# huziqi/NALO-SLAM

Measured on AMD Instinct MI355X. Metric: keyframes/sec, KITTI-00 dense 8-KF photometric BA; pose RMSE vs ref, higher is better.
Workload: dtype f32; 1 GPU; kitti00_8kf; image=1224x368, levels=4, window_frames=8, active_points=2000, residuals=14000, tracked_frames_per_keyframe=3, multi_gpu=replicas (window too small to shard)

## Files before the change

### nalo-slam_amd/csrc/kernels_tracker.hip

```cpp
#include "nalo_internal.h"
#include "reduce.h"
#include "trk_device.h"

namespace nalo {

struct TrkEvalParams {
    TrkLevel L;
    int lvl;
    int i0, i1;
    float RKi[9], t[3], Ki[9];
    float affa, affb, b0, cutoff, maxEnergy;
};
typedef float trk_f4 __attribute__((ext_vector_type(4)));

constexpr int kTrkEvalNT = 512;
constexpr int kTrkEvalNG = kTrkEvalNT / 13;
__global__ __launch_bounds__(kTrkEvalNT) void trk_eval_kernel(TrkEvalParams P, float* __restrict__ partial, unsigned* __restrict__ ticket, double* __restrict__ out, double seq) {
    __shared__ __attribute__((aligned(16))) float smem[(kTrkEvalNT / 4) * (kTrkVals + 1)];
    float acc[kTrkVals];
#pragma unroll
    for (int k = 0; k < kTrkVals; ++k) acc[k] = 0.f;
    const TrkLevel& L = P.L;
    const float wlm3 = (float)(L.wl - 3), hlm3 = (float)(L.hl - 3);
    for (int i = P.i0 + blockIdx.x * blockDim.x + threadIdx.x; i < P.i1; i += gridDim.x * blockDim.x) {
// ... 69 lines not shown
int trk_eval_launch(nalo_ctx* c, int slot_new, int lvl, const float RKi[9], const float t[3], const float Ki[9],
                    float affa, float affb, float b0, float cutoff, float maxEnergy, double out64[64]) {
    TrkEvalParams P;
    P.L = trk_level(c, slot_new, lvl); P.lvl = lvl;
    const bool sharded = c->trk_world > 1 && c->trk_hook;
    P.i0 = sharded ? (int)((long long)P.L.n * c->trk_rank / c->trk_world) : 0;
    P.i1 = sharded ? (int)((long long)P.L.n * (c->trk_rank + 1) / c->trk_world) : P.L.n;
    for (int i = 0; i < 9; ++i) { P.RKi[i] = RKi[i]; P.Ki[i] = Ki[i]; }
    for (int i = 0; i < 3; ++i) P.t[i] = t[i];
    P.affa = affa; P.affb = affb; P.b0 = b0; P.cutoff = cutoff; P.maxEnergy = maxEnergy;
    int nblocks = (P.i1 - P.i0 + kTrkEvalNT - 1) / kTrkEvalNT;
    nblocks = nblocks < 1 ? 1 : (nblocks > 512 ? 512 : nblocks);
    NALO_HIP(c, c->trk_partial.reserve((size_t)2048 * 64));
    if (!c->trk_ticket.p) { NALO_HIP(c, c->trk_ticket.reserve(4)); NALO_HIP(c, hipMemsetAsync(c->trk_ticket.p, 0, 16, c->stream)); }
    double* const dout = c->trk_out_host.dev;
    const double seq = (double)(++c->trk_seq);
    if (sharded) NALO_HIP(c, c->trk_shard_sums.reserve(64));
    {
        ProfScope ps(c, "trk_eval");
        trk_eval_kernel<<<nblocks, kTrkEvalNT, 0, c->stream>>>(P, c->trk_partial.p, c->trk_ticket.p, sharded ? c->trk_shard_sums.p : dout, sharded ? 0.0 : seq);
    }
    if (sharded) {
        if (!c->trk_hook_stream_ordered) NALO_HIP(c, hipStreamSynchronize(c->stream));
        c->trk_hook(c->trk_hook_user, c->trk_shard_sums.p, kTrkVals);
        if (c->xchg_failed) return NALO_ERR_HIP;
        trk_publish_kernel<<<1, 64, 0, c->stream>>>(c->trk_shard_sums.p, dout, seq);
    }
    NALO_HIP(c, hipGetLastError());
    if (!poll_flag(c, &c->trk_out_host.p[63], seq)) return NALO_ERR_HIP;
    std::memcpy(out64, c->trk_out_host.p, sizeof(double) * kTrkVals);
    return NALO_OK;
}

__global__ __launch_bounds__(256) void trk_scatter_kernel(const float* __restrict__ Ku, const float* __restrict__ Kv, const float* __restrict__ nid,
                                                          const float* __restrict__ HdiF, int n, int w0, int h0, float* __restrict__ idepth, float* __restrict__ wsum, int* __restrict__ cnt) {
    const int i = blockIdx.x * blockDim.x + threadIdx.x;
    if (i >= n) return;
    const int u = (int)(Ku[i] + 0.5f), v = (int)(Kv[i] + 0.5f);
    if (u < 0 || v < 0 || u >= w0 || v >= h0) return;
    const float weight = sqrtf((float)(1e-3 / ((double)HdiF[i] + 1e-12)));
    atomicAdd(idepth + u + w0 * v, nid[i] * weight);
    atomicAdd(wsum + u + w0 * v, weight);
    atomicAdd(cnt + u + w0 * v, 1);
}
constexpr int kScatterFixLds = 4096;
struct ScatterListLds {
    int* p;
    __device__ int ld(int k) const { return p[k]; }
    __device__ void st(int k, int v) const { p[k] = v; }
};
struct ScatterListGlobal {
    int* p;
    __device__ int ld(int k) const { return __hip_atomic_load(p + k, __ATOMIC_RELAXED, __HIP_MEMORY_SCOPE_AGENT); }
    __device__ void st(int k, int v) const { __hip_atomic_store(p + k, v, __ATOMIC_RELAXED, __HIP_MEMORY_SCOPE_AGENT); }
};
template <int NT, class List>
__device__ __forceinline__ void trk_scatter_fix_rounds(List list, int m, const float* __restrict__ Ku, const float* __restrict__ Kv, const float* __restrict__ nid,
                                                       const float* __restrict__ HdiF, int w0, float* __restrict__ idepth, float* __restrict__ wsum, int* __restrict__ cnt) {
    const int tid = threadIdx.x;
    for (int k = tid; k < m; k += NT) {
        const int i = list.ld(k), p = (int)(Ku[i] + 0.5f) + w0 * (int)(Kv[i] + 0.5f);
        atomicExch(idepth + p, 0.f); atomicExch(wsum + p, 0.f); atomicExch(cnt + p, 0x7fffffff);
    }
    __syncthreads();
    for (int k = tid; k < m; k += NT) { const int i = list.ld(k); atomicMin(cnt + (int)(Ku[i] + 0.5f) + w0 * (int)(Kv[i] + 0.5f), i); }
    __syncthreads();
    for (int round = 0; round < m; ++round) {
        bool any = false;
        for (int k = tid; k < m; k += NT) {
            const int i = list.ld(k);
            if (i < 0) continue;
            const int p = (int)(Ku[i] + 0.5f) + w0 * (int)(Kv[i] + 0.5f);
            if (__hip_atomic_load(cnt + p, __ATOMIC_RELAXED, __HIP_MEMORY_SCOPE_AGENT) == i) {
                const float weight = sqrtf((float)(1e-3 / ((double)HdiF[i] + 1e-12)));
                atomicAdd(idepth + p, __fmul_rn(nid[i], weight)); atomicAdd(wsum + p, weight);
                list.st(k, -1 - i);
            } else any = true;
        }
        __syncthreads();
        if (!__syncthreads_or(any)) break;
        for (int k = tid; k < m; k += NT) { const int i = list.ld(k); if (i < 0) { const int j = -1 - i, p = (int)(Ku[j] + 0.5f) + w0 * (int)(Kv[j] + 0.5f); atomicCAS(cnt + p, j, 0x7fffffff); } }
        __syncthreads();
        for (int k = tid; k < m; k += NT) { const int i = list.ld(k); if (i >= 0) atomicMin(cnt + (int)(Ku[i] + 0.5f) + w0 * (int)(Kv[i] + 0.5f), i); }
        __syncthreads();
    }
}
template <int NT>
__device__ __forceinline__ void trk_scatter_fix_body(const float* __restrict__ Ku, const float* __restrict__ Kv, const float* __restrict__ nid, const float* __restrict__ HdiF,
                                                     int w0, float* __restrict__ idepth, float* __restrict__ wsum, int* __restrict__ cnt, int* __restrict__ hot, int* slist) {
    const int tid = threadIdx.x;
    const int m = __hip_atomic_load(hot, __ATOMIC_RELAXED, __HIP_MEMORY_SCOPE_AGENT);
    if (m == 0) return;
    __syncthreads();
    if (tid == 0) __hip_atomic_store(hot, 0, __ATOMIC_RELAXED, __HIP_MEMORY_SCOPE_AGENT);
    if (m > kScatterFixLds) { trk_scatter_fix_rounds<NT>(ScatterListGlobal{hot + 2}, m, Ku, Kv, nid, HdiF, w0, idepth, wsum, cnt); return; }
    for (int k = tid; k < m; k += NT) slist[k] = __hip_atomic_load(hot + 2 + k, __ATOMIC_RELAXED, __HIP_MEMORY_SCOPE_AGENT);
    __syncthreads();
    trk_scatter_fix_rounds<NT>(ScatterListLds{slist}, m, Ku, Kv, nid, HdiF, w0, idepth, wsum, cnt);
}
__global__ __launch_bounds__(256) void trk_scatter_hot_kernel(const float* __restrict__ Ku, const float* __restrict__ Kv, const float* __restrict__ nid, const float* __restrict__ HdiF,
                                                              int n, int w0, int h0, float* __restrict__ idepth, float* __restrict__ wsum, int* __restrict__ cnt,
                                                              int* __restrict__ hot ) {
    __shared__ int slist[kScatterFixLds];
    __shared__ int is_last;
    const int i = blockIdx.x * blockDim.x + threadIdx.x;
    if (i < n) {
        const int u = (int)(Ku[i] + 0.5f), v = (int)(Kv[i] + 0.5f);
        if (!(u < 0 || v < 0 || u >= w0 || v >= h0) && __hip_atomic_load(cnt + u + w0 * v, __ATOMIC_RELAXED, __HIP_MEMORY_SCOPE_AGENT) >= 3) {
            const int at = atomicAdd(hot, 1);
            __hip_atomic_store(hot + 2 + at, i, __ATOMIC_RELAXED, __HIP_MEMORY_SCOPE_AGENT);
        }
    }
    __builtin_amdgcn_fence(__ATOMIC_RELEASE, "workgroup");
    __syncthreads();
    if (threadIdx.x == 0) is_last = __hip_atomic_fetch_add((unsigned*)(hot + 1), 1u, __ATOMIC_RELAXED, __HIP_MEMORY_SCOPE_AGENT) == gridDim.x - 1u;
    __syncthreads();
    if (!is_last) return;
    if (threadIdx.x == 0) __hip_atomic_store(hot + 1, 0, __ATOMIC_RELAXED, __HIP_MEMORY_SCOPE_AGENT);
    trk_scatter_fix_body<256>(Ku, Kv, nid, HdiF, w0, idepth, wsum, cnt, hot, slist);
}
struct TrkLevels {
    float *id[NALO_MAX_LEVELS], *ws[NALO_MAX_LEVELS], *wb[NALO_MAX_LEVELS];
    const float4* dI[NALO_MAX_LEVELS];
    float *pu[NALO_MAX_LEVELS], *pv[NALO_MAX_LEVELS], *pid[NALO_MAX_LEVELS], *pcol[NALO_MAX_LEVELS];
    int wl[NALO_MAX_LEVELS], hl[NALO_MAX_LEVELS];
    int blk0[NALO_MAX_LEVELS + 1];
    int scan0[NALO_MAX_LEVELS + 1];
    int L;
};
__global__ __launch_bounds__(256) void trk_zero2_kernel(float* __restrict__ a, float* __restrict__ b, int* __restrict__ cnt, int n) {
    const int i = blockIdx.x * blockDim.x + threadIdx.x;
    if (i < n) { a[i] = 0.f; b[i] = 0.f; cnt[i] = 0; }
    if (i == 0) { cnt[n] = 0; cnt[n + 1] = 0; }
}
__global__ __launch_bounds__(256) void trk_sum_down_all_kernel(TrkLevels P) {
    __shared__ float sid[2][16 * 16], sws[2][16 * 16];
    const int tx = threadIdx.x & 15, ty = threadIdx.x >> 4;
    const int tiles_x = (P.wl[1] + 15) / 16;
    const int bx = blockIdx.x % tiles_x, by = blockIdx.x / tiles_x;
    {
        const int x = bx * 16 + tx, y = by * 16 + ty, w0 = P.wl[0];
        float a = 0.f, b = 0.f;
        if (x < P.wl[1] && y < P.hl[1]) {
            const int o = 2 * x + 2 * y * w0;
            a = P.id[0][o] + P.id[0][o + 1] + P.id[0][o + w0] + P.id[0][o + w0 + 1];
            b = P.ws[0][o] + P.ws[0][o + 1] + P.ws[0][o + w0] + P.ws[0][o + w0 + 1];
            P.id[1][x + y * P.wl[1]] = a; P.ws[1][x + y * P.wl[1]] = b;
        }
        sid[0][ty * 16 + tx] = a; sws[0][ty * 16 + tx] = b;
    }
    int side = 16, cur = 0;
    for (int l = 2; l < P.L; ++l) {
        __syncthreads();
        const int ps = side; side >>= 1;
        if (side == 0) break;
        if (tx < side && ty < side) {
            const int x = bx * side + tx, y = by * side + ty, o = 2 * tx + 2 * ty * ps;
            const float a = sid[cur][o] + sid[cur][o + 1] + sid[cur][o + ps] + sid[cur][o + ps + 1];
            const float b = sws[cur][o] + sws[cur][o + 1] + sws[cur][o + ps] + sws[cur][o + ps + 1];
            if (x < P.wl[l] && y < P.hl[l]) { P.id[l][x + y * P.wl[l]] = a; P.ws[l][x + y * P.wl[l]] = b; }
            sid[cur ^ 1][ty * side + tx] = a; sws[cur ^ 1][ty * side + tx] = b;
        }
        cur ^= 1;
    }
}
__global__ __launch_bounds__(256) void trk_dilate_all_kernel(TrkLevels P) {
    int l = 0;
    while (l + 1 < P.L && (int)blockIdx.x >= P.blk0[l + 1]) ++l;
    const int wl = P.wl[l], npx = wl * P.hl[l];
    const int i = (blockIdx.x - P.blk0[l]) * blockDim.x + threadIdx.x;
    if (i >= npx) return;
    float* __restrict__ id = P.id[l]; const float* __restrict__ bak = P.ws[l]; float* __restrict__ out = P.wb[l];
    const float own = bak[i];
    float res = own;
    if (i >= wl && i < npx - wl && !(own > 0)) {
        const int diag = l < 2;
        const int o0 = diag ? 1 + wl : 1, o1 = diag ? -1 - wl : -1, o2 = diag ? wl - 1 : wl, o3 = diag ? -wl + 1 : -wl;
        float sum = 0, num = 0, numn = 0;
#define NALO_TAP(o) { const int j = i + (o); if (j >= 0 && j < npx) { const float b = bak[j]; if (b > 0) { sum += id[j]; num += b; numn++; } } }
        NALO_TAP(o0) NALO_TAP(o1) NALO_TAP(o2) NALO_TAP(o3)
#undef NALO_TAP
        if (numn > 0) { id[i] = sum / numn; res = num / numn; }
    }
    out[i] = res;
}
constexpr int kCompactChunk = 2048;
template <int WRITE>
__global__ __launch_bounds__(256) void trk_compact_all_kernel(TrkLevels P, int* __restrict__ scan) {
    constexpr int R = kCompactChunk / 256;
    __shared__ int cnt[R * 4 + 1];
    int l = 0;
    while (l + 1 < P.L && (int)blockIdx.x >= P.blk0[l + 1]) ++l;
    const int chunk = blockIdx.x - P.blk0[l], nb = P.blk0[l + 1] - P.blk0[l];
    const int wl = P.wl[l], hl = P.hl[l];
    float* __restrict__ id = P.id[l]; float* __restrict__ ws = P.wb[l]; const float4* __restrict__ dIref = P.dI[l];
    int* counts = scan + P.scan0[l]; const int* offsets = counts + nb;
    const int iw = wl - 4, ih = hl - 4, total = iw * ih;
    const int base = chunk * kCompactChunk;
    const int lane = threadIdx.x & 63, wave = threadIdx.x >> 6;
    int idx[R]; float wsv[R];
#pragma unroll
    for (int r = 0; r < R; ++r) {
        const int e = base + r * 256 + threadIdx.x;
        idx[r] = -1; wsv[r] = 0.f;
        if (e < total) { const int y = e / iw, x = e - y * iw; idx[r] = (x + 2) + (y + 2) * wl; wsv[r] = ws[idx[r]]; }
    }
    float val[R], col[R]; bool keep[R];
#pragma unroll
    for (int r = 0; r < R; ++r) {
        val[r] = 0.f; col[r] = 0.f; keep[r] = false;
        if (idx[r] >= 0 && wsv[r] > 0) { val[r] = id[idx[r]]; col[r] = dIref[idx[r]].x; }
    }
    int rank[R];
#pragma unroll
    for (int r = 0; r < R; ++r) {
        if (idx[r] >= 0 && wsv[r] > 0) { val[r] = val[r] / wsv[r]; keep[r] = isfinite(col[r]) && (val[r] > 0); }
        const unsigned long long m = __ballot(keep[r]);
        rank[r] = __popcll(m & ((1ull << lane) - 1ull));
        if (lane == 0) cnt[r * 4 + wave] = __popcll(m);
    }
    __syncthreads();
    if (!WRITE) {
        if (threadIdx.x == 0) { int t = 0; for (int k = 0; k < R * 4; ++k) t += cnt[k]; counts[chunk] = t; }
        return;
    }
    if (threadIdx.x < 64) {
        const int v = lane < R * 4 ? cnt[lane] : 0;
        int inc = v;
#pragma unroll
        for (int o = 1; o < 64; o <<= 1) { const int t = __shfl_up(inc, o); if (lane >= o) inc += t; }
        if (lane < R * 4) cnt[lane] = inc - v;
    }
    __syncthreads();
    const int first = offsets[chunk];
#pragma unroll
    for (int r = 0; r < R; ++r) {
        const int i = idx[r];
        if (i < 0) continue;
        if (wsv[r] > 0) {
            id[i] = keep[r] ? val[r] : -1.f; if (keep[r]) ws[i] = 1.f;
            if (keep[r]) {
                const int o = first + cnt[r * 4 + wave] + rank[r];
                const int y = i / wl, x = i - y * wl;
                P.pu[l][o] = (float)x; P.pv[l][o] = (float)y; P.pid[l][o] = val[r]; P.pcol[l][o] = col[r];
            }
        } else { id[i] = -1.f; ws[i] = 1.f; }
    }
}
__global__ __launch_bounds__(1024) void trk_scan_all_kernel(TrkLevels P, int* __restrict__ scan, double* __restrict__ out, double seq) {
    __shared__ int part[4][4];
    const int grp = threadIdx.x >> 8, t = threadIdx.x & 255, lane = threadIdx.x & 63, wave = t >> 6;
    for (int l0 = 0; l0 < P.L; l0 += 4) {
        const int l = l0 + grp;
        const bool on = l < P.L;
        const int nb = on ? P.blk0[l + 1] - P.blk0[l] : 0;
        const int* counts = scan + (on ? P.scan0[l] : 0); int* offsets = scan + (on ? P.scan0[l] : 0) + nb;
        const int per = (nb + 255) / 256, lo = min(t * per, nb), hi = min(lo + per, nb);
        int s = 0;
        for (int i = lo; i < hi; ++i) s += counts[i];
        int v = s;
#pragma unroll
        for (int off = 1; off < 64; off <<= 1) { const int nbv = __shfl_up(v, off); if (lane >= off) v += nbv; }
        if (lane == 63) part[grp][wave] = v;
        __syncthreads();
        int wpre = 0, tot = 0;
        for (int k = 0; k < 4; ++k) { const int pv = part[grp][k]; if (k < wave) wpre += pv; tot += pv; }
        int run = wpre + v - s;
        for (int i = lo; i < hi; ++i) { offsets[i] = run; run += counts[i]; }
        if (on && t == 0) { offsets[nb] = tot; out[l] = (double)tot; }
        __syncthreads();
    }
    __threadfence_system();
    __syncthreads();
    if (threadIdx.x == 0) __hip_atomic_store(&out[NALO_MAX_LEVELS], seq, __ATOMIC_RELEASE, __HIP_MEMORY_SCOPE_SYSTEM);
}

__global__ __launch_bounds__(1024) void trk_append_plane_kernel(const float* __restrict__ mask, const float4* __restrict__ dIref, int w, float d0, float d1, float d2, float dis,
                                                                float Ki00, float Ki02, float Ki11, float Ki12, float refColor, int x0, int nx, int y0, int ny, int n0,
                                                                float* __restrict__ pu, float* __restrict__ pv, float* __restrict__ pid, float* __restrict__ pcol, int* __restrict__ n_out) {
    __shared__ int wave_cnt[16];
    __shared__ int base_s;
    const int tid = threadIdx.x, lane = tid & 63, wv = tid >> 6;
    if (tid == 0) { base_s = 0; pu[n0] = 0.f; pv[n0] = 0.f; pid[n0] = 0.f; pcol[n0] = 0.f; }
    __syncthreads();
    const float t0 = d0 * Ki00 + d1 * 0.f + d2 * 0.f, t1 = d0 * 0.f + d1 * Ki11 + d2 * 0.f, t2 = d0 * Ki02 + d1 * Ki12 + d2 * 1.f;
    const int total = nx * ny;
    for (int c0 = 0; c0 < total; c0 += 1024) {
        const int j = c0 + tid;
        bool take = false; int x = 0, y = 0;
        if (j < total) { x = x0 + 5 * (j / ny); y = y0 + 5 * (j % ny); take = mask[x + y * w] == refColor; }
        const unsigned long long b = __ballot(take);
        if (lane == 0) wave_cnt[wv] = __popcll(b);
        __syncthreads();
        int off = base_s;
        for (int k = 0; k < wv; ++k) off += wave_cnt[k];
        if (take) {
            const int at = n0 + 1 + off + __popcll(b & ((1ull << lane) - 1ull));
            float nid = t0 * (float)x + t1 * (float)y + t2 * 1.f;
            nid /= -dis;
            pu[at] = (float)x; pv[at] = (float)y; pid[at] = nid; pcol[at] = dIref[x + y * w].x;
        }
        __syncthreads();
        if (tid == 0) { int s = 0; for (int k = 0; k < 16; ++k) s += wave_cnt[k]; base_s += s; }
        __syncthreads();
    }
    if (tid == 0) *n_out = base_s;
}
int trk_append_plane_launch(nalo_ctx* c, const float* mask, const float4* dIref, const float dir[3], float dis, float refColor, int x0, int nx, int y0, int ny, int n0, int* n_dev) {
    const float fx = c->fx[0], fy = c->fy[0], cx = c->cx[0], cy = c->cy[0];
    trk_append_plane_kernel<<<1, 1024, 0, c->stream>>>(mask, dIref, c->w, dir[0], dir[1], dir[2], dis, 1.0f / fx, -cx / fx, 1.0f / fy, -cy / fy, refColor, x0, nx, y0, ny, n0,
                                                       c->pc_u[0].p, c->pc_v[0].p, c->pc_id[0].p, c->pc_col[0].p, n_dev);
    NALO_HIP(c, hipGetLastError());
    return NALO_OK;
}

int trk_build_ref(nalo_ctx* c, int n, const float* dKu, const float* dKv, const float* dId, const float* dHdi) {
    const int L = c->levels;
    TrkLevels P;
    std::memset(&P, 0, sizeof(P));
    P.L = L;
    int dil_blocks = 0, cmp_blocks = 0, scan_total = 0;
    int dil0[NALO_MAX_LEVELS + 1] = {0}, cmp0[NALO_MAX_LEVELS + 1] = {0};
    for (int l = 0; l < L; ++l) {
        const size_t npx = (size_t)c->wl[l] * c->hl[l];
        NALO_HIP(c, c->trk_idepth[l].reserve(npx)); NALO_HIP(c, c->trk_wsum[l].reserve(npx)); NALO_HIP(c, c->trk_wbak[l].reserve(npx));
        NALO_HIP(c, c->pc_u[l].reserve(npx)); NALO_HIP(c, c->pc_v[l].reserve(npx)); NALO_HIP(c, c->pc_id[l].reserve(npx)); NALO_HIP(c, c->pc_col[l].reserve(npx));
        P.id[l] = c->trk_idepth[l].p; P.ws[l] = c->trk_wsum[l].p; P.wb[l] = c->trk_wbak[l].p; P.dI[l] = c->slots[c->slot_ref].dI[l].p;
        P.pu[l] = c->pc_u[l].p; P.pv[l] = c->pc_v[l].p; P.pid[l] = c->pc_id[l].p; P.pcol[l] = c->pc_col[l].p;
        P.wl[l] = c->wl[l]; P.hl[l] = c->hl[l];
        dil0[l] = dil_blocks; dil_blocks += (int)((npx + 255) / 256);
        const int total = (c->wl[l] - 4) * (c->hl[l] - 4);
        const int nb = total > 0 ? (total + kCompactChunk - 1) / kCompactChunk : 0;
        cmp0[l] = cmp_blocks; cmp_blocks += nb;
        P.scan0[l] = scan_total; scan_total += 2 * nb + 2;
    }
    dil0[L] = dil_blocks; cmp0[L] = cmp_blocks; P.scan0[L] = scan_total;
    NALO_HIP(c, c->scan_tmp.reserve((size_t)scan_total));
    const int n0 = c->wl[0] * c->hl[0];
    NALO_HIP(c, c->trk_cnt.reserve((size_t)n0 + 2 + std::max(n, 0)));
    trk_zero2_kernel<<<(n0 + 255) / 256, 256, 0, c->stream>>>(P.id[0], P.ws[0], c->trk_cnt.p, n0);
    if (n > 0) {
        trk_scatter_kernel<<<(n + 255) / 256, 256, 0, c->stream>>>(dKu, dKv, dId, dHdi, n, c->wl[0], c->hl[0], P.id[0], P.ws[0], c->trk_cnt.p);
        trk_scatter_hot_kernel<<<(n + 255) / 256, 256, 0, c->stream>>>(dKu, dKv, dId, dHdi, n, c->wl[0], c->hl[0], P.id[0], P.ws[0], c->trk_cnt.p, c->trk_cnt.p + n0);
    }
    if (L > 1) trk_sum_down_all_kernel<<<((c->wl[1] + 15) / 16) * ((c->hl[1] + 15) / 16), 256, 0, c->stream>>>(P);
    for (int l = 0; l <= L; ++l) P.blk0[l] = dil0[l];
    trk_dilate_all_kernel<<<dil_blocks, 256, 0, c->stream>>>(P);
    for (int l = 0; l <= L; ++l) P.blk0[l] = cmp0[l];
    double* const dout = c->trk_out_host.dev;
    const double seq = (double)(++c->trk_seq);
    if (cmp_blocks > 0) trk_compact_all_kernel<0><<<cmp_blocks, 256, 0, c->stream>>>(P, c->scan_tmp.p);
    trk_scan_all_kernel<<<1, 1024, 0, c->stream>>>(P, c->scan_tmp.p, dout + 96, seq);
    if (cmp_blocks > 0) trk_compact_all_kernel<1><<<cmp_blocks, 256, 0, c->stream>>>(P, c->scan_tmp.p);
    NALO_HIP(c, hipGetLastError());
    for (int l = 0; l < L; ++l) std::swap(c->trk_wsum[l], c->trk_wbak[l]);
    if (!poll_flag(c, &c->trk_out_host.p[96 + NALO_MAX_LEVELS], seq)) return NALO_ERR_HIP;
    for (int l = 0; l < L; ++l) c->pc_n[l] = (int)c->trk_out_host.p[96 + l];
    return NALO_OK;
}

}
```

### nalo-slam_amd/csrc/nalo_internal.h

```cpp
#pragma once
#include <hip/hip_runtime.h>
#include <cstdint>
#include <cstdio>
#include <cstdlib>
#include <cstring>
#include <map>
#include <string>
#include <utility>
#include <vector>
#include <chrono>

#include "../../include/nalo_gpu.h"
#include "host_math.h"
#include "ref_constants.h"

namespace nalo {

template <typename T>
struct DevBuf {
    T* p = nullptr;
    size_t cap = 0;
    DevBuf() = default;
    DevBuf(const DevBuf&) = delete;
    DevBuf& operator=(const DevBuf&) = delete;
// ... 61 lines not shown
    DevBuf<float> absg[NALO_MAX_LEVELS];
    DevBuf<float> mask;
    DevBuf<uint8_t> bgr;
    bool valid = false;
    Event ev_up;
    DevBuf<uint8_t> raw;
    DevBuf<float> dI0t; bool tiled_valid = false;
};

struct ProfEntry { double ms = 0; int n = 0; std::vector<std::pair<hipEvent_t, hipEvent_t>> pending; std::vector<float> samples; };

struct BAWindow;
struct PixSel;
struct Initializer;

}

struct nalo_ctx {
    int device = 0;
    int w = 0, h = 0, levels = 0;
    int wl[NALO_MAX_LEVELS], hl[NALO_MAX_LEVELS];
    float fx[NALO_MAX_LEVELS], fy[NALO_MAX_LEVELS], cx[NALO_MAX_LEVELS], cy[NALO_MAX_LEVELS];
    float K0[4];
    nalo::Stream stream, side, copy;
    nalo::Event ev_main;
    nalo::DevBuf<float> gamma_dev;
    float gamma_last[256]; bool gamma_have = false;
    int und_wOrg = 0, und_hOrg = 0, und_photometric = 0, und_GDepth = 0; bool und_set = false, und_remap = false, und_vig = false;
    nalo::DevBuf<float> und_G, und_vinv, und_rxy; nalo::DevBuf<uint8_t> und_raw, und_mask, und_bgr;
    std::string err;
    std::vector<nalo::FrameSlot> slots;

    int slot_ref = -1;
    nalo::DevBuf<float> trk_idepth[NALO_MAX_LEVELS], trk_wsum[NALO_MAX_LEVELS], trk_wbak[NALO_MAX_LEVELS];
    nalo::DevBuf<float> pc_u[NALO_MAX_LEVELS], pc_v[NALO_MAX_LEVELS], pc_id[NALO_MAX_LEVELS], pc_col[NALO_MAX_LEVELS];
    int pc_n[NALO_MAX_LEVELS] = {};
    nalo::DevBuf<float> trk_partial;
    nalo::DevBuf<unsigned> trk_ticket;
    nalo::DevBuf<float> ref_res; int ref_res_n = -1;
    nalo::DevBuf<double> trk_out;
    nalo::HostBuf<double> trk_out_host;
    unsigned long long trk_seq = 0;
    nalo::DevBuf<unsigned long long> lm_partial;
    unsigned long long lm_launches = 0;
    int lm_evals_lvl[5] = {};
    int trk_cfg[9] = {};
    int trk_rank = 0, trk_world = 1; nalo_allreduce_fn trk_hook = nullptr; void* trk_hook_user = nullptr; bool trk_hook_stream_ordered = false;
    nalo::DevBuf<double> trk_shard_sums;
    bool lm_host_only = false;
    nalo::DevBuf<int> scan_tmp;
    nalo::DevBuf<unsigned long long> dense_lb;
    nalo::DevBuf<int> trk_cnt;
    nalo::DevBuf<float> upload_tmp;
    nalo::HostBuf<float> pinned_f;
    nalo::HostBuf<float> imm_host; nalo::DevBuf<float> imm_dev;
    nalo::DevBuf<float> imm_res; int imm_res_n = 0, imm_res_maxhost = -1;
    nalo::DevBuf<float> imm_type; bool imm_type_set = false; float imm_type_max = 0;
    nalo::DevBuf<int> imm_act; int imm_act_stats[4] = {};

    nalo::BAWindow* ba = nullptr;
    nalo::PixSel* pixsel = nullptr;
    void* rccl = nullptr;
    bool xchg_failed = false;
    nalo::Initializer* init = nullptr;
    nalo_settings set = {1, nalo::kAffineOptModeA, nalo::kAffineOptModeB, 1};

    bool host_timing = false;
    std::map<std::string, std::pair<double, long>> host_t;

    int inject_lm_lost_block = 0, inject_gated_solve = 0;

    bool prof_on = false;
    std::string prof_only;
    int prof_every = 1; unsigned prof_tick = 0;
    std::vector<hipEvent_t> prof_pool;
    std::map<std::string, nalo::ProfEntry> prof;
};

namespace nalo {

inline int fail(nalo_ctx* c, int code, const std::string& msg) { if (c) c->err = msg; return code; }
#define NALO_HIP(ctx, expr)                                                                          \
    do {                                                                                             \
        hipError_t e__ = (expr);                                                                     \
        if (e__ != hipSuccess)                                                                       \
// ... 104 lines not shown
```

Before: 934.4 keyframes/s.

## Fuse tracker reference build into fewer kernels with decoupled-lookback compaction

Rebuilds the tracker reference-depth pipeline. The scatter and hot-pixel fix are merged into one kernel for small point counts, with the hot list only built when colliding pixels exist. Dilation, the two compaction passes and the scan become a single finish kernel that orders chunks with a ticket and chains prefix offsets through lookback words. Level-0 accumulation buffers are double-buffered so the finish kernel clears the next set, which removes the separate zeroing launch. This cuts launch count and global round trips in trk_build_ref. In exchange it adds spin-waiting between blocks, bounded by a poll limit that reports failure, and more complex host state tracking.

After: 920.3 keyframes/s. -1.5%, worse.

```diff
diff --git a/nalo-slam_amd/csrc/kernels_tracker.hip b/nalo-slam_amd/csrc/kernels_tracker.hip
--- a/nalo-slam_amd/csrc/kernels_tracker.hip
+++ b/nalo-slam_amd/csrc/kernels_tracker.hip
@@ -125,18 +125,9 @@
     return NALO_OK;
 }
 
-__global__ __launch_bounds__(256) void trk_scatter_kernel(const float* __restrict__ Ku, const float* __restrict__ Kv, const float* __restrict__ nid,
-                                                          const float* __restrict__ HdiF, int n, int w0, int h0, float* __restrict__ idepth, float* __restrict__ wsum, int* __restrict__ cnt) {
-    const int i = blockIdx.x * blockDim.x + threadIdx.x;
-    if (i >= n) return;
-    const int u = (int)(Ku[i] + 0.5f), v = (int)(Kv[i] + 0.5f);
-    if (u < 0 || v < 0 || u >= w0 || v >= h0) return;
-    const float weight = sqrtf((float)(1e-3 / ((double)HdiF[i] + 1e-12)));
-    atomicAdd(idepth + u + w0 * v, nid[i] * weight);
-    atomicAdd(wsum + u + w0 * v, weight);
-    atomicAdd(cnt + u + w0 * v, 1);
-}
 constexpr int kScatterFixLds = 4096;
+constexpr int kScatterInlineMax = 16384;
+constexpr int kHotCount = 0, kHotListTicket = 1, kHotPixels = 2, kHotTicket = 3, kHotList = 4;
 struct ScatterListLds {
     int* p;
     __device__ int ld(int k) const { return p[k]; }
@@ -182,49 +173,83 @@
 __device__ __forceinline__ void trk_scatter_fix_body(const float* __restrict__ Ku, const float* __restrict__ Kv, const float* __restrict__ nid, const float* __restrict__ HdiF,
                                                      int w0, float* __restrict__ idepth, float* __restrict__ wsum, int* __restrict__ cnt, int* __restrict__ hot, int* slist) {
     const int tid = threadIdx.x;
-    const int m = __hip_atomic_load(hot, __ATOMIC_RELAXED, __HIP_MEMORY_SCOPE_AGENT);
+    const int m = __hip_atomic_load(hot + kHotCount, __ATOMIC_RELAXED, __HIP_MEMORY_SCOPE_AGENT);
     if (m == 0) return;
     __syncthreads();
-    if (tid == 0) __hip_atomic_store(hot, 0, __ATOMIC_RELAXED, __HIP_MEMORY_SCOPE_AGENT);
-    if (m > kScatterFixLds) { trk_scatter_fix_rounds<NT>(ScatterListGlobal{hot + 2}, m, Ku, Kv, nid, HdiF, w0, idepth, wsum, cnt); return; }
-    for (int k = tid; k < m; k += NT) slist[k] = __hip_atomic_load(hot + 2 + k, __ATOMIC_RELAXED, __HIP_MEMORY_SCOPE_AGENT);
+    if (tid == 0) __hip_atomic_store(hot + kHotCount, 0, __ATOMIC_RELAXED, __HIP_MEMORY_SCOPE_AGENT);
+    if (m > kScatterFixLds) { trk_scatter_fix_rounds<NT>(ScatterListGlobal{hot + kHotList}, m, Ku, Kv, nid, HdiF, w0, idepth, wsum, cnt); return; }
+    for (int k = tid; k < m; k += NT) slist[k] = __hip_atomic_load(hot + kHotList + k, __ATOMIC_RELAXED, __HIP_MEMORY_SCOPE_AGENT);
     __syncthreads();
     trk_scatter_fix_rounds<NT>(ScatterListLds{slist}, m, Ku, Kv, nid, HdiF, w0, idepth, wsum, cnt);
 }
-__global__ __launch_bounds__(256) void trk_scatter_hot_kernel(const float* __restrict__ Ku, const float* __restrict__ Kv, const float* __restrict__ nid, const float* __restrict__ HdiF,
-                                                              int n, int w0, int h0, float* __restrict__ idepth, float* __restrict__ wsum, int* __restrict__ cnt,
-                                                              int* __restrict__ hot ) {
-    __shared__ int slist[kScatterFixLds];
-    __shared__ int is_last;
+__device__ __forceinline__ void trk_scatter_list(int i, const float* __restrict__ Ku, const float* __restrict__ Kv, int w0, int h0, const int* __restrict__ cnt, int* __restrict__ hot) {
+    const int u = (int)(Ku[i] + 0.5f), v = (int)(Kv[i] + 0.5f);
+    if (!(u < 0 || v < 0 || u >= w0 || v >= h0) && __hip_atomic_load(cnt + u + w0 * v, __ATOMIC_RELAXED, __HIP_MEMORY_SCOPE_AGENT) >= 3) {
+        const int at = atomicAdd(hot + kHotCount, 1);
+        __hip_atomic_store(hot + kHotList + at, i, __ATOMIC_RELAXED, __HIP_MEMORY_SCOPE_AGENT);
+    }
+}
+__device__ __forceinline__ bool trk_last_ticket(unsigned* ticket, unsigned total, int* s_flag) {
+    __builtin_amdgcn_fence(__ATOMIC_RELEASE, "workgroup");
+    __syncthreads();
+    if (threadIdx.x == 0) *s_flag = __hip_atomic_fetch_add(ticket, 1u, __ATOMIC_ACQ_REL, __HIP_MEMORY_SCOPE_AGENT) == total - 1u;
+    __syncthreads();
+    return *s_flag != 0;
+}
+template <bool INLINE_FIX>
+__global__ __launch_bounds__(256) void trk_scatter_kernel(const float* __restrict__ Ku, const float* __restrict__ Kv, const float* __restrict__ nid,
+                                                          const float* __restrict__ HdiF, int n, int w0, int h0, float* __restrict__ idepth, float* __restrict__ wsum, int* __restrict__ cnt,
+                                                          int* __restrict__ hot) {
     const int i = blockIdx.x * blockDim.x + threadIdx.x;
     if (i < n) {
         const int u = (int)(Ku[i] + 0.5f), v = (int)(Kv[i] + 0.5f);
-        if (!(u < 0 || v < 0 || u >= w0 || v >= h0) && __hip_atomic_load(cnt + u + w0 * v, __ATOMIC_RELAXED, __HIP_MEMORY_SCOPE_AGENT) >= 3) {
-            const int at = atomicAdd(hot, 1);
-            __hip_atomic_store(hot + 2 + at, i, __ATOMIC_RELAXED, __HIP_MEMORY_SCOPE_AGENT);
-        }
-    }
-    __builtin_amdgcn_fence(__ATOMIC_RELEASE, "workgroup");
-    __syncthreads();
-    if (threadIdx.x == 0) is_last = __hip_atomic_fetch_add((unsigned*)(hot + 1), 1u, __ATOMIC_RELAXED, __HIP_MEMORY_SCOPE_AGENT) == gridDim.x - 1u;
-    __syncthreads();
-    if (!is_last) return;
-    if (threadIdx.x == 0) __hip_atomic_store(hot + 1, 0, __ATOMIC_RELAXED, __HIP_MEMORY_SCOPE_AGENT);
+        if (!(u < 0 || v < 0 || u >= w0 || v >= h0)) {
+            const float weight = sqrtf((float)(1e-3 / ((double)HdiF[i] + 1e-12)));
+            atomicAdd(idepth + u + w0 * v, nid[i] * weight);
+            atomicAdd(wsum + u + w0 * v, weight);
+            if (atomicAdd(cnt + u + w0 * v, 1) == 2) atomicAdd(hot + kHotPixels, 1);
+        }
+    }
+    if (!INLINE_FIX) return;
+    __shared__ int slist[kScatterFixLds];
+    __shared__ int is_last;
+    if (!trk_last_ticket((unsigned*)(hot + kHotTicket), gridDim.x, &is_last)) return;
+    if (threadIdx.x == 0) __hip_atomic_store(hot + kHotTicket, 0, __ATOMIC_RELAXED, __HIP_MEMORY_SCOPE_AGENT);
+    if (__hip_atomic_load(hot + kHotPixels, __ATOMIC_RELAXED, __HIP_MEMORY_SCOPE_AGENT) == 0) return;
+    __syncthreads();
+    if (threadIdx.x == 0) __hip_atomic_store(hot + kHotPixels, 0, __ATOMIC_RELAXED, __HIP_MEMORY_SCOPE_AGENT);
+    for (int k = threadIdx.x; k < n; k += 256) trk_scatter_list(k, Ku, Kv, w0, h0, cnt, hot);
+    __builtin_amdgcn_fence(__ATOMIC_RELEASE, "agent");
+    __syncthreads();
     trk_scatter_fix_body<256>(Ku, Kv, nid, HdiF, w0, idepth, wsum, cnt, hot, slist);
 }
+__global__ __launch_bounds__(256) void trk_scatter_hot_kernel(const float* __restrict__ Ku, const float* __restrict__ Kv, const float* __restrict__ nid, const float* __restrict__ HdiF,
+                                                              int n, int w0, int h0, float* __restrict__ idepth, float* __restrict__ wsum, int* __restrict__ cnt, int* __restrict__ hot) {
+    __shared__ int slist[kScatterFixLds];
+    __shared__ int is_last;
+    if (__hip_atomic_load(hot + kHotPixels, __ATOMIC_RELAXED, __HIP_MEMORY_SCOPE_AGENT) == 0) return;
+    const int i = blockIdx.x * blockDim.x + threadIdx.x;
+    if (i < n) trk_scatter_list(i, Ku, Kv, w0, h0, cnt, hot);
+    if (!trk_last_ticket((unsigned*)(hot + kHotListTicket), gridDim.x, &is_last)) return;
+    if (threadIdx.x == 0) {
+        __hip_atomic_store(hot + kHotListTicket, 0, __ATOMIC_RELAXED, __HIP_MEMORY_SCOPE_AGENT);
+        __hip_atomic_store(hot + kHotPixels, 0, __ATOMIC_RELAXED, __HIP_MEMORY_SCOPE_AGENT);
+    }
+    trk_scatter_fix_body<256>(Ku, Kv, nid, HdiF, w0, idepth, wsum, cnt, hot, slist);
+}
 struct TrkLevels {
-    float *id[NALO_MAX_LEVELS], *ws[NALO_MAX_LEVELS], *wb[NALO_MAX_LEVELS];
+    float *sid[NALO_MAX_LEVELS], *sws[NALO_MAX_LEVELS];
+    float *id[NALO_MAX_LEVELS], *ws[NALO_MAX_LEVELS];
     const float4* dI[NALO_MAX_LEVELS];
     float *pu[NALO_MAX_LEVELS], *pv[NALO_MAX_LEVELS], *pid[NALO_MAX_LEVELS], *pcol[NALO_MAX_LEVELS];
     int wl[NALO_MAX_LEVELS], hl[NALO_MAX_LEVELS];
     int blk0[NALO_MAX_LEVELS + 1];
-    int scan0[NALO_MAX_LEVELS + 1];
+    int brd0[NALO_MAX_LEVELS + 1];
     int L;
 };
-__global__ __launch_bounds__(256) void trk_zero2_kernel(float* __restrict__ a, float* __restrict__ b, int* __restrict__ cnt, int n) {
+__global__ __launch_bounds__(256) void trk_zero4_kernel(float4* __restrict__ p, int n4) {
     const int i = blockIdx.x * blockDim.x + threadIdx.x;
-    if (i < n) { a[i] = 0.f; b[i] = 0.f; cnt[i] = 0; }
-    if (i == 0) { cnt[n] = 0; cnt[n + 1] = 0; }
+    if (i < n4) p[i] = make_float4(0.f, 0.f, 0.f, 0.f);
 }
 __global__ __launch_bounds__(256) void trk_sum_down_all_kernel(TrkLevels P) {
     __shared__ float sid[2][16 * 16], sws[2][16 * 16];
@@ -236,9 +261,9 @@
         float a = 0.f, b = 0.f;
         if (x < P.wl[1] && y < P.hl[1]) {
             const int o = 2 * x + 2 * y * w0;
-            a = P.id[0][o] + P.id[0][o + 1] + P.id[0][o + w0] + P.id[0][o + w0 + 1];
-            b = P.ws[0][o] + P.ws[0][o + 1] + P.ws[0][o + w0] + P.ws[0][o + w0 + 1];
-            P.id[1][x + y * P.wl[1]] = a; P.ws[1][x + y * P.wl[1]] = b;
+            a = P.sid[0][o] + P.sid[0][o + 1] + P.sid[0][o + w0] + P.sid[0][o + w0 + 1];
+            b = P.sws[0][o] + P.sws[0][o + 1] + P.sws[0][o + w0] + P.sws[0][o + w0 + 1];
+            P.sid[1][x + y * P.wl[1]] = a; P.sws[1][x + y * P.wl[1]] = b;
         }
         sid[0][ty * 16 + tx] = a; sws[0][ty * 16 + tx] = b;
     }
@@ -251,121 +276,187 @@
             const int x = bx * side + tx, y = by * side + ty, o = 2 * tx + 2 * ty * ps;
             const float a = sid[cur][o] + sid[cur][o + 1] + sid[cur][o + ps] + sid[cur][o + ps + 1];
             const float b = sws[cur][o] + sws[cur][o + 1] + sws[cur][o + ps] + sws[cur][o + ps + 1];
-            if (x < P.wl[l] && y < P.hl[l]) { P.id[l][x + y * P.wl[l]] = a; P.ws[l][x + y * P.wl[l]] = b; }
+            if (x < P.wl[l] && y < P.hl[l]) { P.sid[l][x + y * P.wl[l]] = a; P.sws[l][x + y * P.wl[l]] = b; }
             sid[cur ^ 1][ty * side + tx] = a; sws[cur ^ 1][ty * side + tx] = b;
         }
         cur ^= 1;
     }
 }
-__global__ __launch_bounds__(256) void trk_dilate_all_kernel(TrkLevels P) {
-    int l = 0;
-    while (l + 1 < P.L && (int)blockIdx.x >= P.blk0[l + 1]) ++l;
-    const int wl = P.wl[l], npx = wl * P.hl[l];
-    const int i = (blockIdx.x - P.blk0[l]) * blockDim.x + threadIdx.x;
-    if (i >= npx) return;
-    float* __restrict__ id = P.id[l]; const float* __restrict__ bak = P.ws[l]; float* __restrict__ out = P.wb[l];
-    const float own = bak[i];
-    float res = own;
-    if (i >= wl && i < npx - wl && !(own > 0)) {
-        const int diag = l < 2;
-        const int o0 = diag ? 1 + wl : 1, o1 = diag ? -1 - wl : -1, o2 = diag ? wl - 1 : wl, o3 = diag ? -wl + 1 : -wl;
-        float sum = 0, num = 0, numn = 0;
-#define NALO_TAP(o) { const int j = i + (o); if (j >= 0 && j < npx) { const float b = bak[j]; if (b > 0) { sum += id[j]; num += b; numn++; } } }
-        NALO_TAP(o0) NALO_TAP(o1) NALO_TAP(o2) NALO_TAP(o3)
-#undef NALO_TAP
-        if (numn > 0) { id[i] = sum / numn; res = num / numn; }
-    }
-    out[i] = res;
-}
 constexpr int kCompactChunk = 2048;
-template <int WRITE>
-__global__ __launch_bounds__(256) void trk_compact_all_kernel(TrkLevels P, int* __restrict__ scan) {
+constexpr unsigned kRefPollSpins = 1u << 21;
+struct TrkFinish {
+    unsigned long long* words;
+    unsigned long long* ctl;
+    unsigned tag;
+    float4* clear; int clear_n4;
+    double* out; double seq;
+};
+__device__ __forceinline__ void trk_dilate_offsets(int l, int wl, int o[4]) {
+    const bool diag = l < 2;
+    o[0] = diag ? 1 + wl : 1; o[1] = diag ? -1 - wl : -1; o[2] = diag ? wl - 1 : wl; o[3] = diag ? -wl + 1 : -wl;
+}
+__device__ __forceinline__ void trk_dilate_px(float own, float own_id, bool dil, const float t[4], const float a[4], float& idd, float& wsd) {
+    idd = own_id; wsd = own;
+    if (!dil) return;
+    float sum = 0, num = 0, numn = 0;
+#pragma unroll
+    for (int k = 0; k < 4; ++k) if (t[k] > 0) { sum += a[k]; num += t[k]; numn++; }
+    if (numn > 0) { idd = sum / numn; wsd = num / numn; }
+}
+__global__ __launch_bounds__(256) void trk_finish_all_kernel(TrkLevels P, TrkFinish F) {
     constexpr int R = kCompactChunk / 256;
     __shared__ int cnt[R * 4 + 1];
-    int l = 0;
-    while (l + 1 < P.L && (int)blockIdx.x >= P.blk0[l + 1]) ++l;
-    const int chunk = blockIdx.x - P.blk0[l], nb = P.blk0[l + 1] - P.blk0[l];
-    const int wl = P.wl[l], hl = P.hl[l];
-    float* __restrict__ id = P.id[l]; float* __restrict__ ws = P.wb[l]; const float4* __restrict__ dIref = P.dI[l];
-    int* counts = scan + P.scan0[l]; const int* offsets = counts + nb;
-    const int iw = wl - 4, ih = hl - 4, total = iw * ih;
-    const int base = chunk * kCompactChunk;
-    const int lane = threadIdx.x & 63, wave = threadIdx.x >> 6;
-    int idx[R]; float wsv[R];
-#pragma unroll
-    for (int r = 0; r < R; ++r) {
-        const int e = base + r * 256 + threadIdx.x;
-        idx[r] = -1; wsv[r] = 0.f;
-        if (e < total) { const int y = e / iw, x = e - y * iw; idx[r] = (x + 2) + (y + 2) * wl; wsv[r] = ws[idx[r]]; }
-    }
-    float val[R], col[R]; bool keep[R];
-#pragma unroll
-    for (int r = 0; r < R; ++r) {
-        val[r] = 0.f; col[r] = 0.f; keep[r] = false;
-        if (idx[r] >= 0 && wsv[r] > 0) { val[r] = id[idx[r]]; col[r] = dIref[idx[r]].x; }
-    }
-    int rank[R];
-#pragma unroll
-    for (int r = 0; r < R; ++r) {
-        if (idx[r] >= 0 && wsv[r] > 0) { val[r] = val[r] / wsv[r]; keep[r] = isfinite(col[r]) && (val[r] > 0); }
-        const unsigned long long m = __ballot(keep[r]);
-        rank[r] = __popcll(m & ((1ull << lane) - 1ull));
-        if (lane == 0) cnt[r * 4 + wave] = __popcll(m);
-    }
-    __syncthreads();
-    if (!WRITE) {
-        if (threadIdx.x == 0) { int t = 0; for (int k = 0; k < R * 4; ++k) t += cnt[k]; counts[chunk] = t; }
-        return;
-    }
-    if (threadIdx.x < 64) {
-        const int v = lane < R * 4 ? cnt[lane] : 0;
-        int inc = v;
-#pragma unroll
-        for (int o = 1; o < 64; o <<= 1) { const int t = __shfl_up(inc, o); if (lane >= o) inc += t; }
-        if (lane < R * 4) cnt[lane] = inc - v;
-    }
-    __syncthreads();
-    const int first = offsets[chunk];
-#pragma unroll
-    for (int r = 0; r < R; ++r) {
-        const int i = idx[r];
-        if (i < 0) continue;
-        if (wsv[r] > 0) {
-            id[i] = keep[r] ? val[r] : -1.f; if (keep[r]) ws[i] = 1.f;
-            if (keep[r]) {
-                const int o = first + cnt[r * 4 + wave] + rank[r];
-                const int y = i / wl, x = i - y * wl;
-                P.pu[l][o] = (float)x; P.pv[l][o] = (float)y; P.pid[l][o] = val[r]; P.pcol[l][o] = col[r];
+    __shared__ int s_order, s_ok, s_part[4];
+    const int tid = threadIdx.x, lane = tid & 63, wave = tid >> 6;
+    {
+        const int per = (F.clear_n4 + (int)gridDim.x - 1) / (int)gridDim.x;
+        const int a = min((int)blockIdx.x * per, F.clear_n4), b = min(a + per, F.clear_n4);
+        for (int i = a + tid; i < b; i += 256) F.clear[i] = make_float4(0.f, 0.f, 0.f, 0.f);
+    }
+    if (tid == 0) { s_order = (int)__hip_atomic_fetch_add(F.ctl, 1ull, __ATOMIC_RELAXED, __HIP_MEMORY_SCOPE_AGENT); s_ok = 1; }
+    __syncthreads();
+    const int order = s_order, nchunks = P.blk0[P.L];
+    bool wrote_total = false, failed = false;
+    if (order < nchunks) {
+        int l = 0;
+        while (l + 1 < P.L && order >= P.blk0[l + 1]) ++l;
+        const int chunk = order - P.blk0[l];
+        const int wl = P.wl[l], hl = P.hl[l];
+        const float* __restrict__ sid = P.sid[l]; const float* __restrict__ bak = P.sws[l]; const float4* __restrict__ dIref = P.dI[l];
+        float* __restrict__ id = P.id[l]; float* __restrict__ ws = P.ws[l];
+        const int iw = wl - 4, total = iw * (hl - 4);
+        const int base = chunk * kCompactChunk;
+        int o[4]; trk_dilate_offsets(l, wl, o);
+        int idx[R]; float own[R], t[R][4];
+#pragma unroll
+        for (int r = 0; r < R; ++r) {
+            const int e = base + r * 256 + tid;
+            idx[r] = -1; own[r] = 0.f;
+#pragma unroll
+            for (int k = 0; k < 4; ++k) t[r][k] = 0.f;
+            if (e < total) {
+                const int y = e / iw, x = e - y * iw, i = (x + 2) + (y + 2) * wl;
+                idx[r] = i; own[r] = bak[i];
+#pragma unroll
+                for (int k = 0; k < 4; ++k) t[r][k] = bak[i + o[k]];
             }
-        } else { id[i] = -1.f; ws[i] = 1.f; }
-    }
-}
-__global__ __launch_bounds__(1024) void trk_scan_all_kernel(TrkLevels P, int* __restrict__ scan, double* __restrict__ out, double seq) {
-    __shared__ int part[4][4];
-    const int grp = threadIdx.x >> 8, t = threadIdx.x & 255, lane = threadIdx.x & 63, wave = t >> 6;
-    for (int l0 = 0; l0 < P.L; l0 += 4) {
-        const int l = l0 + grp;
-        const bool on = l < P.L;
-        const int nb = on ? P.blk0[l + 1] - P.blk0[l] : 0;
-        const int* counts = scan + (on ? P.scan0[l] : 0); int* offsets = scan + (on ? P.scan0[l] : 0) + nb;
-        const int per = (nb + 255) / 256, lo = min(t * per, nb), hi = min(lo + per, nb);
-        int s = 0;
-        for (int i = lo; i < hi; ++i) s += counts[i];
-        int v = s;
-#pragma unroll
-        for (int off = 1; off < 64; off <<= 1) { const int nbv = __shfl_up(v, off); if (lane >= off) v += nbv; }
-        if (lane == 63) part[grp][wave] = v;
-        __syncthreads();
-        int wpre = 0, tot = 0;
-        for (int k = 0; k < 4; ++k) { const int pv = part[grp][k]; if (k < wave) wpre += pv; tot += pv; }
-        int run = wpre + v - s;
-        for (int i = lo; i < hi; ++i) { offsets[i] = run; run += counts[i]; }
-        if (on && t == 0) { offsets[nb] = tot; out[l] = (double)tot; }
-        __syncthreads();
-    }
-    __threadfence_system();
-    __syncthreads();
-    if (threadIdx.x == 0) __hip_atomic_store(&out[NALO_MAX_LEVELS], seq, __ATOMIC_RELEASE, __HIP_MEMORY_SCOPE_SYSTEM);
+        }
+        float oid[R], a[R][4], col[R];
+#pragma unroll
+        for (int r = 0; r < R; ++r) {
+            const int i = idx[r];
+            const bool dil = i >= 0 && !(own[r] > 0);
+            oid[r] = 0.f; col[r] = 0.f;
+            if (i >= 0 && own[r] > 0) oid[r] = sid[i];
+            bool any = i >= 0 && own[r] > 0;
+#pragma unroll
+            for (int k = 0; k < 4; ++k) { a[r][k] = 0.f; if (dil && t[r][k] > 0) { a[r][k] = sid[i + o[k]]; any = true; } }
+            if (any) col[r] = dIref[i].x;
+        }
+        float val[R], wsv[R]; bool keep[R]; int rank[R];
+#pragma unroll
+        for (int r = 0; r < R; ++r) {
+            float idd;
+            trk_dilate_px(own[r], oid[r], idx[r] >= 0 && !(own[r] > 0), t[r], a[r], idd, wsv[r]);
+            val[r] = 0.f; keep[r] = false;
+            if (idx[r] >= 0 && wsv[r] > 0) { val[r] = idd / wsv[r]; keep[r] = isfinite(col[r]) && (val[r] > 0); }
+            const unsigned long long m = __ballot(keep[r]);
+            rank[r] = __popcll(m & ((1ull << lane) - 1ull));
+            if (lane == 0) cnt[r * 4 + wave] = __popcll(m);
+        }
+        __syncthreads();
+        int mine = 0;
+        if (tid < 64) {
+            const int v = lane < R * 4 ? cnt[lane] : 0;
+            int inc = v;
+#pragma unroll
+            for (int s = 1; s < 64; s <<= 1) { const int up = __shfl_up(inc, s); if (lane >= s) inc += up; }
+            mine = __shfl(inc, 63);
+            if (lane == 0) __hip_atomic_store(&F.words[order], ((unsigned long long)F.tag << 32) | (unsigned)mine, __ATOMIC_RELAXED, __HIP_MEMORY_SCOPE_AGENT);
+            if (lane < R * 4) cnt[lane] = inc - v;
+            if (lane == 0) cnt[R * 4] = mine;
+        }
+        int before = 0;
+        {
+            const unsigned long long* wp = F.words + P.blk0[l];
+            bool pending = tid < chunk;
+            for (unsigned spins = 0; pending; ++spins) {
+                pending = false; before = 0;
+                for (int k = tid; k < chunk; k += 256) {
+                    const unsigned long long wv = __hip_atomic_load(&wp[k], __ATOMIC_RELAXED, __HIP_MEMORY_SCOPE_AGENT);
+                    pending |= (unsigned)(wv >> 32) != F.tag;
+                    before += (int)(unsigned)wv;
+                }
+                if (pending) { if (spins > kRefPollSpins) { s_ok = 0; break; } __builtin_amdgcn_s_sleep(1); }
+            }
+#pragma unroll
+            for (int s = 32; s > 0; s >>= 1) before += __shfl_xor(before, s);
+            if (lane == 0) s_part[wave] = before;
+        }
+        __syncthreads();
+        const int first = s_part[0] + s_part[1] + s_part[2] + s_part[3];
+        const bool ok = s_ok != 0;
+#pragma unroll
+        for (int r = 0; r < R; ++r) {
+            const int i = idx[r];
+            if (i < 0) continue;
+            if (wsv[r] > 0) {
+                id[i] = keep[r] ? val[r] : -1.f; ws[i] = keep[r] ? 1.f : wsv[r];
+                if (keep[r] && ok) {
+                    const int at = first + cnt[r * 4 + wave] + rank[r];
+                    const int y = i / wl, x = i - y * wl;
+                    P.pu[l][at] = (float)x; P.pv[l][at] = (float)y; P.pid[l][at] = val[r]; P.pcol[l][at] = col[r];
+                }
+            } else { id[i] = -1.f; ws[i] = 1.f; }
+        }
+        if (tid == 0) {
+            failed = !ok;
+            if (chunk == P.blk0[l + 1] - P.blk0[l] - 1) { __hip_atomic_store(&F.out[l], (double)(first + cnt[R * 4]), __ATOMIC_RELAXED, __HIP_MEMORY_SCOPE_SYSTEM); wrote_total = true; }
+        }
+    } else {
+        const int bi = order - nchunks;
+        int l = 0;
+        while (l + 1 < P.L && bi >= P.brd0[l + 1]) ++l;
+        const int wl = P.wl[l], hl = P.hl[l], npx = wl * hl;
+        const bool interior = wl > 4 && hl > 4;
+        const int nborder = interior ? 4 * wl + 4 * (hl - 4) : npx;
+        const int b = (bi - P.brd0[l]) * 256 + tid;
+        int i = -1;
+        if (b < nborder) {
+            if (!interior || b < 2 * wl) i = b;
+            else if (b < 4 * wl) i = (hl - 4) * wl + b;
+            else { const int k = b - 4 * wl, c4 = k & 3; i = (2 + (k >> 2)) * wl + (c4 < 2 ? c4 : wl - 4 + c4); }
+        }
+        const float* __restrict__ sid = P.sid[l]; const float* __restrict__ bak = P.sws[l];
+        int o[4]; trk_dilate_offsets(l, wl, o);
+        float own = 0.f, own_id = 0.f, t[4] = {0.f, 0.f, 0.f, 0.f}, a[4] = {0.f, 0.f, 0.f, 0.f};
+        const bool range = i >= wl && i < npx - wl;
+        if (i >= 0) {
+            own = bak[i]; own_id = sid[i];
+            if (range) {
+#pragma unroll
+                for (int k = 0; k < 4; ++k) { const int j = i + o[k]; if (j >= 0 && j < npx) t[k] = bak[j]; }
+            }
+        }
+        const bool dil = range && !(own > 0);
+        if (dil) {
+#pragma unroll
+            for (int k = 0; k < 4; ++k) if (t[k] > 0) a[k] = sid[i + o[k]];
+        }
+        float idd, wsd;
+        trk_dilate_px(own, own_id, dil, t, a, idd, wsd);
+        if (i >= 0) { P.id[l][i] = idd; P.ws[l][i] = wsd; }
+    }
+    if (tid != 0) return;
+    if (wrote_total) __threadfence_system();
+    const unsigned long long before_me = __hip_atomic_fetch_add(F.ctl + 1, 1ull | ((unsigned long long)failed << 32), __ATOMIC_RELAXED, __HIP_MEMORY_SCOPE_AGENT);
+    if ((unsigned)before_me != gridDim.x - 1u) return;
+    __hip_atomic_store(F.ctl, 0ull, __ATOMIC_RELAXED, __HIP_MEMORY_SCOPE_AGENT);
+    __hip_atomic_store(F.ctl + 1, 0ull, __ATOMIC_RELAXED, __HIP_MEMORY_SCOPE_AGENT);
+    for (int l = 0; l < P.L; ++l)
+        if (P.blk0[l + 1] == P.blk0[l]) __hip_atomic_store(&F.out[l], 0.0, __ATOMIC_RELAXED, __HIP_MEMORY_SCOPE_SYSTEM);
+    __hip_atomic_store(&F.out[NALO_MAX_LEVELS + 1], (before_me >> 32) != 0 || failed ? 1.0 : 0.0, __ATOMIC_RELAXED, __HIP_MEMORY_SCOPE_SYSTEM);
+    __hip_atomic_store(&F.out[NALO_MAX_LEVELS], F.seq, __ATOMIC_RELEASE, __HIP_MEMORY_SCOPE_SYSTEM);
 }
 
 __global__ __launch_bounds__(1024) void trk_append_plane_kernel(const float* __restrict__ mask, const float4* __restrict__ dIref, int w, float d0, float d1, float d2, float dis,
@@ -412,43 +503,61 @@
     TrkLevels P;
     std::memset(&P, 0, sizeof(P));
     P.L = L;
-    int dil_blocks = 0, cmp_blocks = 0, scan_total = 0;
-    int dil0[NALO_MAX_LEVELS + 1] = {0}, cmp0[NALO_MAX_LEVELS + 1] = {0};
+    const int n0 = c->wl[0] * c->hl[0];
+    const int set_n4 = (3 * n0 + 3) / 4;
+    for (int s = 0; s < 2; ++s)
+        if (c->trk_set[s].cap < (size_t)set_n4 * 4) { NALO_HIP(c, c->trk_set[s].reserve((size_t)set_n4 * 4)); c->trk_set_clean[s] = false; }
+    const int cur = c->trk_set_cur;
+    int chunks = 0, borders = 0;
     for (int l = 0; l < L; ++l) {
         const size_t npx = (size_t)c->wl[l] * c->hl[l];
-        NALO_HIP(c, c->trk_idepth[l].reserve(npx)); NALO_HIP(c, c->trk_wsum[l].reserve(npx)); NALO_HIP(c, c->trk_wbak[l].reserve(npx));
+        NALO_HIP(c, c->trk_idepth[l].reserve(npx)); NALO_HIP(c, c->trk_wsum[l].reserve(npx));
+        if (l > 0) { NALO_HIP(c, c->trk_sum_id[l].reserve(npx)); NALO_HIP(c, c->trk_sum_ws[l].reserve(npx)); }
         NALO_HIP(c, c->pc_u[l].reserve(npx)); NALO_HIP(c, c->pc_v[l].reserve(npx)); NALO_HIP(c, c->pc_id[l].reserve(npx)); NALO_HIP(c, c->pc_col[l].reserve(npx));
-        P.id[l] = c->trk_idepth[l].p; P.ws[l] = c->trk_wsum[l].p; P.wb[l] = c->trk_wbak[l].p; P.dI[l] = c->slots[c->slot_ref].dI[l].p;
+        P.sid[l] = l ? c->trk_sum_id[l].p : c->trk_set[cur].p; P.sws[l] = l ? c->trk_sum_ws[l].p : c->trk_set[cur].p + n0;
+        P.id[l] = c->trk_idepth[l].p; P.ws[l] = c->trk_wsum[l].p; P.dI[l] = c->slots[c->slot_ref].dI[l].p;
         P.pu[l] = c->pc_u[l].p; P.pv[l] = c->pc_v[l].p; P.pid[l] = c->pc_id[l].p; P.pcol[l] = c->pc_col[l].p;
         P.wl[l] = c->wl[l]; P.hl[l] = c->hl[l];
-        dil0[l] = dil_blocks; dil_blocks += (int)((npx + 255) / 256);
-        const int total = (c->wl[l] - 4) * (c->hl[l] - 4);
-        const int nb = total > 0 ? (total + kCompactChunk - 1) / kCompactChunk : 0;
-        cmp0[l] = cmp_blocks; cmp_blocks += nb;
-        P.scan0[l] = scan_total; scan_total += 2 * nb + 2;
-    }
-    dil0[L] = dil_blocks; cmp0[L] = cmp_blocks; P.scan0[L] = scan_total;
-    NALO_HIP(c, c->scan_tmp.reserve((size_t)scan_total));
-    const int n0 = c->wl[0] * c->hl[0];
-    NALO_HIP(c, c->trk_cnt.reserve((size_t)n0 + 2 + std::max(n, 0)));
-    trk_zero2_kernel<<<(n0 + 255) / 256, 256, 0, c->stream>>>(P.id[0], P.ws[0], c->trk_cnt.p, n0);
-    if (n > 0) {
-        trk_scatter_kernel<<<(n + 255) / 256, 256, 0, c->stream>>>(dKu, dKv, dId, dHdi, n, c->wl[0], c->hl[0], P.id[0], P.ws[0], c->trk_cnt.p);
-        trk_scatter_hot_kernel<<<(n + 255) / 256, 256, 0, c->stream>>>(dKu, dKv, dId, dHdi, n, c->wl[0], c->hl[0], P.id[0], P.ws[0], c->trk_cnt.p, c->trk_cnt.p + n0);
-    }
+        const bool interior = c->wl[l] > 4 && c->hl[l] > 4;
+        const size_t total = interior ? (size_t)(c->wl[l] - 4) * (c->hl[l] - 4) : 0;
+        P.blk0[l] = chunks; chunks += (int)((total + kCompactChunk - 1) / kCompactChunk);
+        P.brd0[l] = borders; borders += (int)((npx - total + 255) / 256);
+    }
+    P.blk0[L] = chunks; P.brd0[L] = borders;
+    int* const cnt = reinterpret_cast<int*>(c->trk_set[cur].p + 2 * (size_t)n0);
+    if (c->trk_hot.cap < (size_t)kHotList + std::max(n, 0)) { NALO_HIP(c, c->trk_hot.reserve((size_t)kHotList + n + 1024)); c->trk_ref_ctl_dirty = true; }
+    if (c->trk_ref_words.cap < (size_t)chunks + 1) { NALO_HIP(c, c->trk_ref_words.reserve((size_t)chunks + 1)); c->trk_ref_builds = 0; }
+    NALO_HIP(c, c->trk_ref_ctl.reserve(2));
+    if ((++c->trk_ref_builds & 0xFFFFFFFFull) == 0 || c->trk_ref_builds == 1) {
+        NALO_HIP(c, hipMemsetAsync(c->trk_ref_words.p, 0, c->trk_ref_words.cap * 8, c->stream));
+        if ((c->trk_ref_builds & 0xFFFFFFFFull) == 0) ++c->trk_ref_builds;
+    }
+    if (c->trk_ref_ctl_dirty) {
+        NALO_HIP(c, hipMemsetAsync(c->trk_hot.p, 0, kHotList * sizeof(int), c->stream));
+        NALO_HIP(c, hipMemsetAsync(c->trk_ref_ctl.p, 0, 2 * sizeof(unsigned long long), c->stream));
+    }
+    const bool cur_clean = c->trk_set_clean[cur];
+    c->trk_ref_ctl_dirty = true; c->trk_set_clean[0] = c->trk_set_clean[1] = false;
+    if (!cur_clean) trk_zero4_kernel<<<(set_n4 + 255) / 256, 256, 0, c->stream>>>(reinterpret_cast<float4*>(c->trk_set[cur].p), set_n4);
+    if (n > kScatterInlineMax) {
+        trk_scatter_kernel<false><<<(n + 255) / 256, 256, 0, c->stream>>>(dKu, dKv, dId, dHdi, n, c->wl[0], c->hl[0], P.sid[0], P.sws[0], cnt, c->trk_hot.p);
+        trk_scatter_hot_kernel<<<(n + 255) / 256, 256, 0, c->stream>>>(dKu, dKv, dId, dHdi, n, c->wl[0], c->hl[0], P.sid[0], P.sws[0], cnt, c->trk_hot.p);
+    } else if (n > 0)
+        trk_scatter_kernel<true><<<(n + 255) / 256, 256, 0, c->stream>>>(dKu, dKv, dId, dHdi, n, c->wl[0], c->hl[0], P.sid[0], P.sws[0], cnt, c->trk_hot.p);
     if (L > 1) trk_sum_down_all_kernel<<<((c->wl[1] + 15) / 16) * ((c->hl[1] + 15) / 16), 256, 0, c->stream>>>(P);
-    for (int l = 0; l <= L; ++l) P.blk0[l] = dil0[l];
-    trk_dilate_all_kernel<<<dil_blocks, 256, 0, c->stream>>>(P);
-    for (int l = 0; l <= L; ++l) P.blk0[l] = cmp0[l];
-    double* const dout = c->trk_out_host.dev;
-    const double seq = (double)(++c->trk_seq);
-    if (cmp_blocks > 0) trk_compact_all_kernel<0><<<cmp_blocks, 256, 0, c->stream>>>(P, c->scan_tmp.p);
-    trk_scan_all_kernel<<<1, 1024, 0, c->stream>>>(P, c->scan_tmp.p, dout + 96, seq);
-    if (cmp_blocks > 0) trk_compact_all_kernel<1><<<cmp_blocks, 256, 0, c->stream>>>(P, c->scan_tmp.p);
+    TrkFinish F;
+    F.words = c->trk_ref_words.p; F.ctl = c->trk_ref_ctl.p; F.tag = (unsigned)c->trk_ref_builds;
+    F.clear = reinterpret_cast<float4*>(c->trk_set[cur ^ 1].p); F.clear_n4 = set_n4;
+    F.out = c->trk_out_host.dev + 96; F.seq = (double)(++c->trk_seq);
+    trk_finish_all_kernel<<<chunks + borders, 256, 0, c->stream>>>(P, F);
     NALO_HIP(c, hipGetLastError());
-    for (int l = 0; l < L; ++l) std::swap(c->trk_wsum[l], c->trk_wbak[l]);
-    if (!poll_flag(c, &c->trk_out_host.p[96 + NALO_MAX_LEVELS], seq)) return NALO_ERR_HIP;
-    for (int l = 0; l < L; ++l) c->pc_n[l] = (int)c->trk_out_host.p[96 + l];
+    volatile double* const out = c->trk_out_host.p + 96;
+    if (!poll_flag(c, &out[NALO_MAX_LEVELS], F.seq)) return NALO_ERR_HIP;
+    if (out[NALO_MAX_LEVELS + 1] != 0.0) return fail(c, NALO_ERR_HIP, "trk_build_ref: a compaction chunk waited for its predecessors beyond the poll bound");
+    for (int l = 0; l < L; ++l) c->pc_n[l] = (int)out[l];
+    c->trk_ref_ctl_dirty = false;
+    c->trk_set_clean[cur ^ 1] = true; c->trk_set_clean[cur] = n <= 0;
+    c->trk_set_cur = cur ^ 1;
     return NALO_OK;
 }
 
diff --git a/nalo-slam_amd/csrc/nalo_internal.h b/nalo-slam_amd/csrc/nalo_internal.h
--- a/nalo-slam_amd/csrc/nalo_internal.h
+++ b/nalo-slam_amd/csrc/nalo_internal.h
@@ -117,7 +117,14 @@
     std::vector<nalo::FrameSlot> slots;
 
     int slot_ref = -1;
-    nalo::DevBuf<float> trk_idepth[NALO_MAX_LEVELS], trk_wsum[NALO_MAX_LEVELS], trk_wbak[NALO_MAX_LEVELS];
+    nalo::DevBuf<float> trk_idepth[NALO_MAX_LEVELS], trk_wsum[NALO_MAX_LEVELS];
+    nalo::DevBuf<float> trk_sum_id[NALO_MAX_LEVELS], trk_sum_ws[NALO_MAX_LEVELS];
+    nalo::DevBuf<float> trk_set[2]; bool trk_set_clean[2] = {false, false}; int trk_set_cur = 0;
+    nalo::DevBuf<int> trk_hot;
+    nalo::DevBuf<unsigned long long> trk_ref_words;
+    nalo::DevBuf<unsigned long long> trk_ref_ctl;
+    unsigned long long trk_ref_builds = 0;
+    bool trk_ref_ctl_dirty = true;
     nalo::DevBuf<float> pc_u[NALO_MAX_LEVELS], pc_v[NALO_MAX_LEVELS], pc_id[NALO_MAX_LEVELS], pc_col[NALO_MAX_LEVELS];
     int pc_n[NALO_MAX_LEVELS] = {};
     nalo::DevBuf<float> trk_partial;
@@ -135,7 +142,6 @@
     bool lm_host_only = false;
     nalo::DevBuf<int> scan_tmp;
     nalo::DevBuf<unsigned long long> dense_lb;
-    nalo::DevBuf<int> trk_cnt;
     nalo::DevBuf<float> upload_tmp;
     nalo::HostBuf<float> pinned_f;
     nalo::HostBuf<float> imm_host; nalo::DevBuf<float> imm_dev;
```
